# Harrypotterrrr/DVD-GAN

Measured on AMD Instinct MI355X. Metric: clips/sec per G+Ds+Dt step, 48x64x64 UCF-101 synth, higher is better.
Workload: dtype bf16; 1 GPU; UCF-101-shaped 101-class 48x64x64 clips, G+Ds+Dt hinge step, ch=32, k_sample=8, batch 64/GPU (BASELINE configs[1]); global_batch=64, parallelism=dp1

## Files before the change

dvd_gan_amd/csrc/conv_gb.hip:

```cpp
#include "conv_common.h"

namespace {

#ifndef DVD_GB_EPI_DEEP
#define DVD_GB_EPI_DEEP 0
#endif

constexpr unsigned kRowOOB = 0x80000000u, kStepOOB = 0x40000000u, kRangeCap = 0x3fffffffu;

template <int TM, int WN, int WMV, bool UP2> struct HaloGbCfg {
    static constexpr int PITCH = HaloGeo<UP2>::PITCH;
    static constexpr int NWAVE = WMV * WN;
    static constexpr int PH = WMV * TM * 2;
    static constexpr int HG = UP2 ? ((PH / 2 + 3) * PITCH + 15) / 16 : ((PH + 4) * PITCH + 15) / 16;
    static constexpr int HBYTES = HG * 1024;
    static constexpr int EPI = NWAVE * 32 * 64 * 4;
    static constexpr int LDSB = 2 * HBYTES + 1024 > EPI ? 2 * HBYTES + 1024 : EPI;
};

template <int TM, bool RELU, class LdA, class Next>
__device__ __forceinline__ void gb_step(f32x16 (&acc)[TM][2], const bf16x8 (&b)[2][2], LdA ldA, Next next) {
    constexpr int NU = 2 * TM;
#ifndef DVD_GB_ADEPTH
#define DVD_GB_ADEPTH 2
#endif
    constexpr int AD = DVD_GB_ADEPTH;
    bf16x8 a[NU];
#pragma unroll
    for (int u = 0; u < AD && u < NU; ++u) a[u] = ldA(u);
    __builtin_amdgcn_sched_barrier(0);
#pragma unroll
    for (int u = 0; u < NU; ++u) {
        if (u + AD < NU) a[u + AD] = ldA(u + AD);
        const int kk = u / TM, tm = u % TM;
        if constexpr (RELU) a[u] = __builtin_bit_cast(bf16x8, relu16_bf16(__builtin_bit_cast(u32x4, a[u])));
#pragma unroll
        for (int tn = 0; tn < 2; ++tn)
            acc[tm][tn] = __builtin_amdgcn_mfma_f32_32x32x16_bf16(a[u], b[kk][tn], acc[tm][tn], 0, 0, 0);
        __builtin_amdgcn_sched_barrier(0);
        if (u == 0) {
#ifndef DVD_EXP_NODMA
            next();
#endif
            __builtin_amdgcn_sched_barrier(0);
        }
    }
}

template <int TM, int WN, int WMV, bool RELU, bool UP2, int KS>
__device__ __forceinline__ void conv_halo_gb_tile(const ConvK& p, char* const smem, const int mt, const int nt, const int z, const int ltile) {
    using T = bf16_t;
    using G = HaloGeo<UP2>;
    using Cfg = HaloGbCfg<TM, WN, WMV, UP2>;
    constexpr int NWAVE = Cfg::NWAVE;
    constexpr int PITCH = G::PITCH;
    constexpr int BNt = WN * 64;
    constexpr int PH = Cfg::PH, HG = Cfg::HG, HBYTES = Cfg::HBYTES;
    constexpr int NH = (HG + NWAVE - 1) / NWAVE;
    constexpr int ntap2 = KS * KS;
    constexpr int pad = KS >> 1, cpad = (pad + 1) >> 1;
    constexpr int HWa = UP2 ? ((15 + pad) >> 1) + cpad + 1 : 16 + 2 * pad;
    constexpr int HHa = UP2 ? ((PH - 1 + pad) >> 1) + cpad + 1 : PH + 2 * pad;
    char* const hbuf0 = &smem[0];
    char* const dump = &smem[2 * HBYTES];
    const int tid = threadIdx.x, lane = tid & 63, wave = tid >> 6;
    const int wm = wave / WN, wn = wave % WN;
    const int n0 = nt * BNt;
    const int pw = p.W >> 4, ppf = pw * (p.H / PH);
    const int ft = mt / ppf, pidx = mt - ft * ppf;
    const int y0 = (pidx / pw) * PH, x0 = (pidx % pw) * 16;
    const int nouter = p.kchunks * p.kt;
    const int per = (nouter + p.nsplit - 1) / p.nsplit;
    const int oc_begin = z * per, oc_end = min(nouter, oc_begin + per);
    constexpr unsigned esz = 2;
    const int iy_lo = UP2 ? (y0 >> 1) - cpad : y0 - pad, ix_lo = UP2 ? (x0 >> 1) - cpad : x0 - pad;

    const int wu = __builtin_amdgcn_readfirstlane(wave);
    const int lrow = lane >> 2;
    const unsigned ldb = (unsigned)p.ldi * esz;
    const int tt = p.kt > 1 ? ft % p.T : 0;
    const int base_frame = max(0, ft - (p.kt >> 1));
    const size_t fbytes = (size_t)p.Hin * p.Win * ldb;
    const size_t base_b = (size_t)base_frame * fbytes;
    const size_t left_b = p.in_bytes - base_b;
    const __amdgpu_buffer_rsrc_t rin = __builtin_amdgcn_make_buffer_rsrc(
        (void*)(p.in + base_b), 0, left_b > kRangeCap ? kRangeCap : (unsigned)left_b, 0x00020000);
    const int nb32 = p.nb32;
    const __amdgpu_buffer_rsrc_t rwq = __builtin_amdgcn_make_buffer_rsrc(
        (void*)p.wq, 0, (unsigned)((size_t)p.kt * ntap2 * p.kchunks * nb32 * 2048), 0x00020000);
    auto hrow = [&](int i, int& hy, int& hx) __attribute__((always_inline)) {
        const int h = (i * NWAVE + wu) * 16 + lrow;
        hy = h / PITCH; hx = h - hy * PITCH;
    };
    unsigned hoff[NH];
#pragma unroll
    for (int i = 0; i < NH; ++i) {
        const int g = i * NWAVE + wu;
        int hy, hx;
        hrow(i, hy, hx);
        const int yin = iy_lo + hy, xin = ix_lo + hx;
        const int hq = (lane & 3) ^ G::sw(hy, hx);
        const bool ok = g < HG && hy < HHa && hx < HWa && (unsigned)yin < (unsigned)p.Hin && (unsigned)xin < (unsigned)p.Win;
        hoff[i] = ok ? (unsigned)(yin * p.Win + xin) * ldb + hq * 16 : kRowOOB;
    }
    const bool ragged = (p.C & 31) != 0;
    auto dmaH = [&](int hb, int cc_, int it_) __attribute__((always_inline)) {
        const int dt_ = it_ - (p.kt >> 1);
        const bool ok_ = (unsigned)(tt + dt_) < (unsigned)p.T || p.kt == 1;
        const unsigned ud_ = ok_ ? (unsigned)(ft + dt_ - base_frame) * (unsigned)fbytes + cc_ * 64 : kStepOOB;
        const bool part_ = ragged && cc_ == p.kchunks - 1;
#pragma unroll
        for (int i = 0; i < NH; ++i) {
            const int g = i * NWAVE + wu;
            char* dst_ = g < HG ? hbuf0 + hb * HBYTES + g * 1024 : dump;
            unsigned off_ = hoff[i] + ud_;
            if (part_) {
                int hy, hx;
                hrow(i, hy, hx);
                const int hq = (lane & 3) ^ G::sw(hy, hx);
                off_ = cc_ * 32 + hq * 8 < p.C ? off_ : kRowOOB;
            }
            dma16(rin, dst_, off_);
        }
    };
    const unsigned bvoff = (unsigned)(wn * 2 * 2048 + lane * 16);
    const unsigned bnt = (unsigned)(nt * (BNt / 32)) * 2048u;
    const unsigned brec = (unsigned)nb32 * 2048u;
    const unsigned tapstep = (unsigned)p.kchunks * brec;
    auto ldBq = [&](bf16x8 (&b)[2][2], unsigned rec) __attribute__((always_inline)) {
#pragma unroll
        for (int kk = 0; kk < 2; ++kk)
#pragma unroll
            for (int tn = 0; tn < 2; ++tn)
                b[kk][tn] = __builtin_bit_cast(bf16x8, __builtin_amdgcn_raw_buffer_load_b128(rwq, bvoff, rec + (unsigned)(tn * 2048 + kk * 1024), 0));
    };
    auto rec0 = [&](int cc_, int it_) __attribute__((always_inline)) -> unsigned {
        return ((unsigned)(it_ * ntap2) * p.kchunks + cc_) * brec + bnt;
    };

    f32x16 acc[TM][2];
    {
        const f32x16 zacc = {0.f, 0.f, 0.f, 0.f, 0.f, 0.f, 0.f, 0.f, 0.f, 0.f, 0.f, 0.f, 0.f, 0.f, 0.f, 0.f};
#pragma unroll
        for (int a = 0; a < TM; ++a)
#pragma unroll
            for (int b = 0; b < 2; ++b) acc[a][b] = zacc;
    }
    const int l31 = lane & 31, kh2 = lane >> 5;
    const int px = l31 & 15, py0 = wm * (TM * 2) + (l31 >> 4);
    constexpr int TMSTRIDE = (UP2 ? 1 : 2) * PITCH * 64;
#ifdef DVD_EXP_NOMAIN
    const int nouter_z = 0;
#else
    const int nouter_z = oc_end - oc_begin;
#endif
    if (nouter_z > 0) {
        int m_cc = oc_begin / p.kt, m_it = oc_begin - m_cc * p.kt;
        int h_cc = m_cc, h_it = m_it;
        bf16x8 bq0[2][2], bq1[2][2];
        unsigned rec = rec0(m_cc, m_it);
        dmaH(0, h_cc, h_it);
        if (++h_it == p.kt) { h_it = 0; ++h_cc; }
        ldBq(bq0, rec);
        __builtin_amdgcn_s_waitcnt(0x0070 | (0xf << 8));
        __builtin_amdgcn_s_barrier();
        int hb = 0, iy = 0, left = nouter_z;
        auto row = [&](bf16x8 (&b0)[2][2], bf16x8 (&b1)[2][2]) __attribute__((always_inline)) {
            const bool first = iy == 0, last = iy == KS - 1, more = left > 1;
            const int hy = UP2 ? ((py0 + iy - pad) >> 1) + cpad : py0 + iy;
            const char* const Arow = hbuf0 + hb * HBYTES + hy * (PITCH * 64);
#pragma unroll
            for (int ix = 0; ix < KS; ++ix) {
                const int hx = UP2 ? ((px + ix - pad) >> 1) + cpad : px + ix;
                const int swz = G::sw(hy, hx);
                const char* const Ah = Arow + hx * 64;
                auto ldA = [&](int u) __attribute__((always_inline)) -> bf16x8 {
                    const int kk = u / TM, tm = u % TM, slot = kk * 2 + kh2;
                    const int sl = (UP2 && (tm & 1)) ? (slot ^ 2) : slot;
                    return *reinterpret_cast<const bf16x8*>(Ah + tm * TMSTRIDE + ((sl ^ swz) << 4));
                };
                unsigned nrec = rec + tapstep;
                if (ix == KS - 1 && last) {
                    int n_cc = m_cc, n_it = m_it + 1;
                    if (n_it == p.kt) { n_it = 0; ++n_cc; }
                    nrec = more ? rec0(n_cc, n_it) : rec;
                    m_cc = n_cc; m_it = n_it;
                }
                auto next = [&]() __attribute__((always_inline)) {
                    ldBq((ix & 1) ? b0 : b1, nrec);
                    if (ix == 0 && first && more) { dmaH(hb ^ 1, h_cc, h_it); if (++h_it == p.kt) { h_it = 0; ++h_cc; } }
                };
                gb_step<TM, RELU>(acc, (ix & 1) ? b1 : b0, ldA, next);
                rec = nrec;
            }
            ++iy;
            if (last) {
                iy = 0; hb ^= 1; --left;
                if (more) {
#ifndef DVD_EXP_NOWAIT
                    __builtin_amdgcn_s_waitcnt(0xc07f);
#endif
#ifndef DVD_EXP_NOBAR
                    __builtin_amdgcn_s_barrier();
#endif
                }
            }
        };
        const int nrows = nouter_z * KS;
        int r = 0;
#pragma unroll 1
        for (; r + 1 < nrows; r += 2) { row(bq0, bq1); row(bq1, bq0); }
        if (r < nrows) row(bq0, bq1);
    }
    __syncthreads();

    float* ep = reinterpret_cast<float*>(&smem[0]) + wave * (32 * 64);
    const int ecol = (lane & 7) * 8, erow = lane >> 3;
    const long long frame_row0 = (long long)ft * (p.H * p.W);
    conv_epilogue<T, TM, DVD_GB_EPI_DEEP>(p, acc, ep, lane, n0 + wn * 64 + ecol, z, ltile, frame_row0, [&](int tm, int j) __attribute__((always_inline)) {
        const int pi = wm * (TM * 32) + tm * 32 + j * 8 + erow;
        return (y0 + (pi >> 4)) * p.W + x0 + (pi & 15);
    });
}

__device__ __forceinline__ int xcd_order(int bid, int nwg) {
    const int xcd = bid & 7, qd = nwg >> 3, rr = nwg & 7;
    return (xcd < rr ? xcd * (qd + 1) : rr * (qd + 1) + (xcd - rr) * qd) + (bid >> 3);
}
struct TileMN { int mt, nt; };
__device__ __forceinline__ TileMN tile_of(int nmajor, int tilesN, int t, int ntiles) {
    const int d = nmajor ? ntiles / tilesN : tilesN;
    const int q = t / d, r = t - q * d;
    TileMN o;
    o.mt = nmajor ? r : q; o.nt = nmajor ? q : r;
    return o;
}

template <int TM, int WN, int WMV, bool RELU, bool UP2, int KS>
__global__ __launch_bounds__(256, 2) void conv_halo_gb_kernel(ConvK p) {
    __shared__ __attribute__((aligned(16))) char smem[HaloGbCfg<TM, WN, WMV, UP2>::LDSB];
    const int bid = xcd_order(blockIdx.x, gridDim.x);
    const TileMN t = tile_of(p.nmajor, p.tilesN, bid, gridDim.x);
    conv_halo_gb_tile<TM, WN, WMV, RELU, UP2, KS>(p, smem, t.mt, t.nt, blockIdx.z, (int)blockIdx.x);
}

template <int TM, int S> struct HaloGbsCfg {
    static constexpr int PITCH = S + 4, FR = PITCH * PITCH;
    static constexpr int G = TM * 64 / (S * S);
    static constexpr int HG = (G * FR + 15) / 16;
    static constexpr int HBYTES = HG * 1024;
    static constexpr int EPI = 4 * 32 * 64 * 4;
    static constexpr int LDSB = 2 * HBYTES + 1024 > EPI ? 2 * HBYTES + 1024 : EPI;
};

template <int TM, int S, bool RELU, int KS>
__device__ __forceinline__ void conv_halo_gbs_tile(const ConvK& p, char* const smem, const int mt, const int nt, const int z, const int ltile) {
    using T = bf16_t;
    using Cfg = HaloGbsCfg<TM, S>;
    constexpr int WN = 2, NWAVE = 4, BNt = 128;
    constexpr int PITCH = Cfg::PITCH, FR = Cfg::FR, G = Cfg::G, HG = Cfg::HG, HBYTES = Cfg::HBYTES;
    constexpr int NH = (HG + NWAVE - 1) / NWAVE;
    constexpr int SS = S * S;
    constexpr int ntap2 = KS * KS, pad = KS >> 1, ext = S + 2 * pad;
    char* const hbuf0 = &smem[0];
    char* const dump = &smem[2 * HBYTES];
    const int tid = threadIdx.x, lane = tid & 63, wave = tid >> 6;
    const int wm = wave / WN, wn = wave % WN;
    const int n0 = nt * BNt;
    const int ft0 = mt * G, nframes = p.M / SS;
    const int per = (p.kchunks + p.nsplit - 1) / p.nsplit;
    const int cc_begin = z * per, cc_end = min(p.kchunks, cc_begin + per);
    constexpr unsigned esz = 2;

    const int wu = __builtin_amdgcn_readfirstlane(wave);
    const int lrow = lane >> 2;
    const unsigned ldb = (unsigned)p.ldi * esz;
    const size_t base_b = (size_t)ft0 * SS * ldb;
    const size_t left_b = p.in_bytes - base_b;
    const __amdgpu_buffer_rsrc_t rin = __builtin_amdgcn_make_buffer_rsrc(
        (void*)(p.in + base_b), 0, left_b > kRangeCap ? kRangeCap : (unsigned)left_b, 0x00020000);
    const int nb32 = p.nb32;
    const __amdgpu_buffer_rsrc_t rwq = __builtin_amdgcn_make_buffer_rsrc(
        (void*)p.wq, 0, (unsigned)((size_t)ntap2 * p.kchunks * nb32 * 2048), 0x00020000);
    auto hrow = [&](int i, int& fl, int& hy, int& hx) __attribute__((always_inline)) {
        const int h = (i * NWAVE + wu) * 16 + lrow;
        fl = h / FR;
        const int r = h - fl * FR;
        hy = r / PITCH; hx = r - hy * PITCH;
    };
    unsigned hoff[NH];
#pragma unroll
    for (int i = 0; i < NH; ++i) {
        const int g = i * NWAVE + wu;
        int fl, hy, hx;
        hrow(i, fl, hy, hx);
        const int yin = hy - pad, xin = hx - pad;
        const int hq = (lane & 3) ^ (hy & 3);
        const bool ok = g < HG && fl < G && ft0 + fl < nframes && hy < ext && hx < ext && (unsigned)yin < (unsigned)S && (unsigned)xin < (unsigned)S;
        hoff[i] = ok ? (unsigned)((fl * S + yin) * S + xin) * ldb + hq * 16 : kRowOOB;
    }
    const bool ragged = (p.C & 31) != 0;
    auto dmaH = [&](int hb, int cc_) __attribute__((always_inline)) {
        const bool part_ = ragged && cc_ == p.kchunks - 1;
#pragma unroll
        for (int i = 0; i < NH; ++i) {
            const int g = i * NWAVE + wu;
            char* dst_ = g < HG ? hbuf0 + hb * HBYTES + g * 1024 : dump;
            unsigned off_ = hoff[i] + cc_ * 64;
            if (part_) {
                int fl, hy, hx;
                hrow(i, fl, hy, hx);
                const int hq = (lane & 3) ^ (hy & 3);
                off_ = cc_ * 32 + hq * 8 < p.C ? off_ : kRowOOB;
            }
            dma16(rin, dst_, off_);
        }
    };
    const unsigned bvoff = (unsigned)(wn * 2 * 2048 + lane * 16);
    const unsigned bnt = (unsigned)(nt * (BNt / 32)) * 2048u;
    const unsigned brec = (unsigned)nb32 * 2048u;
    const unsigned tapstep = (unsigned)p.kchunks * brec;
    auto ldBq = [&](bf16x8 (&b)[2][2], unsigned rec) __attribute__((always_inline)) {
#pragma unroll
        for (int kk = 0; kk < 2; ++kk)
#pragma unroll
            for (int tn = 0; tn < 2; ++tn)
                b[kk][tn] = __builtin_bit_cast(bf16x8, __builtin_amdgcn_raw_buffer_load_b128(rwq, bvoff, rec + (unsigned)(tn * 2048 + kk * 1024), 0));
    };

    f32x16 acc[TM][2];
    {
        const f32x16 zacc = {0.f, 0.f, 0.f, 0.f, 0.f, 0.f, 0.f, 0.f, 0.f, 0.f, 0.f, 0.f, 0.f, 0.f, 0.f, 0.f};
#pragma unroll
        for (int a = 0; a < TM; ++a)
#pragma unroll
            for (int b = 0; b < 2; ++b) acc[a][b] = zacc;
    }
    const int l31 = lane & 31, kh2 = lane >> 5;
    const int pi0 = wm * (TM * 32) + l31;
    const int f0 = pi0 / SS, y0 = (pi0 % SS) / S, x0 = pi0 % S;
    const int arow0 = f0 * FR + y0 * PITCH + x0;
    auto tmoff = [](int tm) constexpr -> int { return S == 8 ? ((tm >> 1) * FR + (tm & 1) * 4 * PITCH) * 64 : tm * 2 * FR * 64; };
#ifdef DVD_EXP_NOMAIN
    const int nch = 0;
#else
    const int nch = cc_end - cc_begin;
#endif
    if (nch > 0) {
        unsigned rec = (unsigned)cc_begin * brec + bnt;
        bf16x8 bq0[2][2], bq1[2][2];
        dmaH(0, cc_begin);
        ldBq(bq0, rec);
        __builtin_amdgcn_s_waitcnt(0x0070 | (0xf << 8));
        __builtin_amdgcn_s_barrier();
        int hb = 0, iy = 0, cc = cc_begin;
        auto row = [&](bf16x8 (&b0)[2][2], bf16x8 (&b1)[2][2]) __attribute__((always_inline)) {
            const bool first = iy == 0, last = iy == KS - 1, more = cc + 1 < cc_end;
            const int swz = (y0 + iy) & 3;
            const char* const Arow = hbuf0 + hb * HBYTES + (arow0 + iy * PITCH) * 64;
#pragma unroll
            for (int ix = 0; ix < KS; ++ix) {
                const char* const Ah = Arow + ix * 64;
                auto ldA = [&](int u) __attribute__((always_inline)) -> bf16x8 {
                    const int kk = u / TM, tm = u % TM, slot = kk * 2 + kh2;
                    return *reinterpret_cast<const bf16x8*>(Ah + tmoff(tm) + ((slot ^ swz) << 4));
                };
                unsigned nrec = rec + tapstep;
                if (ix == KS - 1 && last) nrec = more ? (unsigned)(cc + 1) * brec + bnt : rec;
                auto next = [&]() __attribute__((always_inline)) {
                    ldBq((ix & 1) ? b0 : b1, nrec);
                    if (ix == 0 && first && more) dmaH(hb ^ 1, cc + 1);
                };
                gb_step<TM, RELU>(acc, (ix & 1) ? b1 : b0, ldA, next);
                rec = nrec;
            }
            ++iy;
            if (last) {
                iy = 0; hb ^= 1; ++cc;
                if (more) {
                    __builtin_amdgcn_s_waitcnt(0xc07f);
                    __builtin_amdgcn_s_barrier();
                }
            }
        };
        const int nrows = nch * KS;
        int r = 0;
#pragma unroll 1
        for (; r + 1 < nrows; r += 2) { row(bq0, bq1); row(bq1, bq0); }
        if (r < nrows) row(bq0, bq1);
    }
    __syncthreads();

    float* ep = reinterpret_cast<float*>(&smem[0]) + wave * (32 * 64);
    const int ecol = (lane & 7) * 8, erow = lane >> 3;
    const long long row0 = (long long)ft0 * SS;
    conv_epilogue<T, TM, DVD_GB_EPI_DEEP>(p, acc, ep, lane, n0 + wn * 64 + ecol, z, ltile, row0, [&](int tm, int j) __attribute__((always_inline)) {
        const int pi = wm * (TM * 32) + tm * 32 + j * 8 + erow;
        return row0 + pi < p.M ? pi : -1;
    });
}

template <int TM, int S, bool RELU, int KS>
__global__ __launch_bounds__(256, 2) void conv_halo_gbs_kernel(ConvK p) {
    __shared__ __attribute__((aligned(16))) char smem[HaloGbsCfg<TM, S>::LDSB];
    const int bid = xcd_order(blockIdx.x, gridDim.x);
    const TileMN t = tile_of(p.nmajor, p.tilesN, bid, gridDim.x);
    conv_halo_gbs_tile<TM, S, RELU, KS>(p, smem, t.mt, t.nt, blockIdx.z, (int)blockIdx.x);
}

template <class TileFn>
__device__ __forceinline__ void group_dispatch(const ConvGroup& grp, TileFn fn) {
    const int x = blockIdx.x & 7;
    int rem = blockIdx.x >> 3;
    auto share = [&](int m) __attribute__((always_inline)) -> int { const int w = grp.wgs[m]; return (w >> 3) + (x < (w & 7) ? 1 : 0); };
    const int m0 = grp.order[0], m1 = grp.n > 1 ? grp.order[1] : m0;
    const int s0 = share(m0), s1 = grp.n > 1 ? share(m1) : 0;
    const int h0 = min(grp.head, s0), h1 = min(grp.head, s1);
    int g = -1, off = 0;
    if (rem < h0) { g = m0; off = rem; }
    else if ((rem -= h0) < h1) { g = m1; off = rem; }
    else if ((rem -= h1) < s0 - h0) { g = m0; off = h0 + rem; }
    else if ((rem -= s0 - h0) < s1 - h1) { g = m1; off = h1 + rem; }
    else {
        rem -= s1 - h1;
        for (int k = 2; k < grp.n; ++k) {
            const int m = grp.order[k], s = share(m);
            if (rem < s) { g = m; off = rem; break; }
            rem -= s;
        }
    }
    if (g < 0) return;
    const int w = grp.wgs[g];
    const int local = x * (w >> 3) + min(x, w & 7) + off;
    const ConvK& p = grp.c[g];
    const int t = local / p.nsplit, z = local - t * p.nsplit;
    const TileMN mn = tile_of(p.nmajor, p.tilesN, t, w / p.nsplit);
    fn(p, mn.mt, mn.nt, z, t);
}

template <int TM, int WN, int WMV>
__global__ __launch_bounds__(256, 2) void conv_group_gb_kernel(ConvGroup grp) {
    __shared__ __attribute__((aligned(16))) char smem[HaloGbCfg<TM, WN, WMV, false>::LDSB];
    group_dispatch(grp, [&](const ConvK& p, int mt, int nt, int z, int t) __attribute__((always_inline)) {
        if (p.kh == 5) conv_halo_gb_tile<TM, WN, WMV, false, false, 5>(p, smem, mt, nt, z, t);
        else conv_halo_gb_tile<TM, WN, WMV, false, false, 3>(p, smem, mt, nt, z, t);
    });
}

template <int TM, int S>
__global__ __launch_bounds__(256, 2) void conv_group_gbs_kernel(ConvGroup grp) {
    __shared__ __attribute__((aligned(16))) char smem[HaloGbsCfg<TM, S>::LDSB];
    group_dispatch(grp, [&](const ConvK& p, int mt, int nt, int z, int t) __attribute__((always_inline)) {
        if (p.kh == 5) conv_halo_gbs_tile<TM, S, false, 5>(p, smem, mt, nt, z, t);
        else conv_halo_gbs_tile<TM, S, false, 3>(p, smem, mt, nt, z, t);
    });
}

}

namespace dvdk {
#define GB(R, C, KS, RL, UP) cv_key(CV_HALO_L2, 0, R, C, KS, RL, UP)
#define GBS(F, R, KS, RL) cv_key(F, 0, R, 128, KS, RL, 0)
static const ConvRow kGbRows[] = {
#ifdef DVD_GB_PROBE
    {GB(256, 128, 5, 0, 0), conv_halo_gb_kernel<4, 2, 2, false, false, 5>}, {GBS(CV_FRAME8, 128, 3, 0), conv_halo_gbs_kernel<2, 8, false, 3>},
#else
    {GB(256, 128, 3, 0, 0), conv_halo_gb_kernel<4, 2, 2, false, false, 3>}, {GB(256, 128, 3, 1, 0), conv_halo_gb_kernel<4, 2, 2, true, false, 3>},
    {GB(256, 128, 3, 0, 1), conv_halo_gb_kernel<4, 2, 2, false, true, 3>},  {GB(256, 128, 3, 1, 1), conv_halo_gb_kernel<4, 2, 2, true, true, 3>},
    {GB(256, 128, 5, 0, 0), conv_halo_gb_kernel<4, 2, 2, false, false, 5>}, {GB(256, 128, 5, 1, 0), conv_halo_gb_kernel<4, 2, 2, true, false, 5>},
    {GB(256, 128, 5, 0, 1), conv_halo_gb_kernel<4, 2, 2, false, true, 5>},  {GB(256, 128, 5, 1, 1), conv_halo_gb_kernel<4, 2, 2, true, true, 5>},
    {GB(128, 128, 3, 0, 0), conv_halo_gb_kernel<2, 2, 2, false, false, 3>}, {GB(128, 128, 3, 1, 0), conv_halo_gb_kernel<2, 2, 2, true, false, 3>},
    {GB(128, 128, 3, 0, 1), conv_halo_gb_kernel<2, 2, 2, false, true, 3>},  {GB(128, 128, 3, 1, 1), conv_halo_gb_kernel<2, 2, 2, true, true, 3>},
    {GB(128, 128, 5, 0, 0), conv_halo_gb_kernel<2, 2, 2, false, false, 5>}, {GB(128, 128, 5, 1, 0), conv_halo_gb_kernel<2, 2, 2, true, false, 5>},
    {GB(128, 128, 5, 0, 1), conv_halo_gb_kernel<2, 2, 2, false, true, 5>},  {GB(128, 128, 5, 1, 1), conv_halo_gb_kernel<2, 2, 2, true, true, 5>},
    {GB(256, 64, 3, 0, 0), conv_halo_gb_kernel<2, 1, 4, false, false, 3>},  {GB(256, 64, 3, 1, 0), conv_halo_gb_kernel<2, 1, 4, true, false, 3>},
    {GB(256, 64, 3, 0, 1), conv_halo_gb_kernel<2, 1, 4, false, true, 3>},   {GB(256, 64, 3, 1, 1), conv_halo_gb_kernel<2, 1, 4, true, true, 3>},
    {GB(256, 64, 5, 0, 0), conv_halo_gb_kernel<2, 1, 4, false, false, 5>},  {GB(256, 64, 5, 1, 0), conv_halo_gb_kernel<2, 1, 4, true, false, 5>},
    {GB(256, 64, 5, 0, 1), conv_halo_gb_kernel<2, 1, 4, false, true, 5>},   {GB(256, 64, 5, 1, 1), conv_halo_gb_kernel<2, 1, 4, true, true, 5>},
    {GBS(CV_FRAME8, 256, 3, 0), conv_halo_gbs_kernel<4, 8, false, 3>},      {GBS(CV_FRAME8, 256, 3, 1), conv_halo_gbs_kernel<4, 8, true, 3>},
    {GBS(CV_FRAME8, 256, 5, 0), conv_halo_gbs_kernel<4, 8, false, 5>},      {GBS(CV_FRAME8, 256, 5, 1), conv_halo_gbs_kernel<4, 8, true, 5>},
    {GBS(CV_FRAME8, 128, 3, 0), conv_halo_gbs_kernel<2, 8, false, 3>},      {GBS(CV_FRAME8, 128, 3, 1), conv_halo_gbs_kernel<2, 8, true, 3>},
    {GBS(CV_FRAME8, 128, 5, 0), conv_halo_gbs_kernel<2, 8, false, 5>},      {GBS(CV_FRAME8, 128, 5, 1), conv_halo_gbs_kernel<2, 8, true, 5>},
    {GBS(CV_FRAME4, 128, 3, 0), conv_halo_gbs_kernel<2, 4, false, 3>},      {GBS(CV_FRAME4, 128, 3, 1), conv_halo_gbs_kernel<2, 4, true, 3>},
    {GBS(CV_FRAME4, 128, 5, 0), conv_halo_gbs_kernel<2, 4, false, 5>},      {GBS(CV_FRAME4, 128, 5, 1), conv_halo_gbs_kernel<2, 4, true, 5>},
#endif
};
#undef GB
#undef GBS
bool launch_gb(unsigned key, const ConvK& p, dim3 grid, hipStream_t st) { return cv_launch_row(kGbRows, (int)(sizeof kGbRows / sizeof kGbRows[0]), key, p, grid, 256, st); }
static void (*const kGroupKernel[])(ConvGroup) = {
#ifdef DVD_GB_PROBE
    conv_group_gb_kernel<4, 2, 2>, conv_group_gb_kernel<4, 2, 2>, conv_group_gb_kernel<4, 2, 2>, conv_group_gb_kernel<4, 2, 2>, conv_group_gb_kernel<4, 2, 2>,
#else
    conv_group_gb_kernel<4, 2, 2>, conv_group_gb_kernel<2, 2, 2>, conv_group_gbs_kernel<4, 8>, conv_group_gbs_kernel<2, 8>, conv_group_gbs_kernel<2, 4>,
#endif
};
static_assert(sizeof kGroupKernel / sizeof kGroupKernel[0] == kGroupKinds, "one kernel per row of kGroupKind");
void launch_group(const ConvGroup& grp, int kind, hipStream_t st) { kGroupKernel[kind]<<<dim3(grp.nslots), 256, 0, st>>>(grp); }
}
```

Measured before the change: 145.1 clips/s.

## Remap small-frame conv tiles to whole image lines and skip all-padding tap rows

Reorganizes the small-frame (S=4/8) halo conv kernel so each 32-row MFMA sub-tile covers whole image lines across frames, using a new compile-time row map. With that layout, per-wave kernel-row ranges and per-row sub-tile masks are computed at compile time, so MFMAs and B loads for taps that only read zero padding are skipped. The chunk loop is fully unrolled per wave-row with a triple-buffered B register set and wave-specific specializations. The changes are meant to remove wasted MFMA work on padding at small spatial sizes, at the cost of more code size, register pressure and a changed LDS swizzle and epilogue mapping.

```diff
diff --git a/dvd_gan_amd/csrc/conv_gb.hip b/dvd_gan_amd/csrc/conv_gb.hip
--- a/dvd_gan_amd/csrc/conv_gb.hip
+++ b/dvd_gan_amd/csrc/conv_gb.hip
@@ -1,10 +1,18 @@
+#include <type_traits>
+#include <utility>
+
 #include "conv_common.h"
+#include "gbs_rowmap.h"
 
 namespace {
 
 #ifndef DVD_GB_EPI_DEEP
 #define DVD_GB_EPI_DEEP 0
 #endif
+
+template <class F, int... I>
+__device__ __forceinline__ void static_for_seq(F&& f, std::integer_sequence<int, I...>) { (f(std::integral_constant<int, I>{}), ...); }
+template <int N, class F> __device__ __forceinline__ void static_for(F&& f) { static_for_seq(f, std::make_integer_sequence<int, N>{}); }
 
 constexpr unsigned kRowOOB = 0x80000000u, kStepOOB = 0x40000000u, kRangeCap = 0x3fffffffu;
 
@@ -18,21 +26,22 @@
     static constexpr int LDSB = 2 * HBYTES + 1024 > EPI ? 2 * HBYTES + 1024 : EPI;
 };
 
-template <int TM, bool RELU, class LdA, class Next>
+template <int TM, int T0, int NT, bool RELU, class LdA, class Next>
 __device__ __forceinline__ void gb_step(f32x16 (&acc)[TM][2], const bf16x8 (&b)[2][2], LdA ldA, Next next) {
-    constexpr int NU = 2 * TM;
+    static_assert(T0 >= 0 && NT >= 1 && T0 + NT <= TM, "sub-tile range");
+    constexpr int NU = 2 * NT;
 #ifndef DVD_GB_ADEPTH
 #define DVD_GB_ADEPTH 2
 #endif
     constexpr int AD = DVD_GB_ADEPTH;
     bf16x8 a[NU];
 #pragma unroll
-    for (int u = 0; u < AD && u < NU; ++u) a[u] = ldA(u);
+    for (int u = 0; u < AD && u < NU; ++u) a[u] = ldA(u / NT, T0 + u % NT);
     __builtin_amdgcn_sched_barrier(0);
 #pragma unroll
     for (int u = 0; u < NU; ++u) {
-        if (u + AD < NU) a[u + AD] = ldA(u + AD);
-        const int kk = u / TM, tm = u % TM;
+        if (u + AD < NU) a[u + AD] = ldA((u + AD) / NT, T0 + (u + AD) % NT);
+        const int kk = u / NT, tm = T0 + u % NT;
         if constexpr (RELU) a[u] = __builtin_bit_cast(bf16x8, relu16_bf16(__builtin_bit_cast(u32x4, a[u])));
 #pragma unroll
         for (int tn = 0; tn < 2; ++tn)
@@ -174,8 +183,8 @@
                 const int hx = UP2 ? ((px + ix - pad) >> 1) + cpad : px + ix;
                 const int swz = G::sw(hy, hx);
                 const char* const Ah = Arow + hx * 64;
-                auto ldA = [&](int u) __attribute__((always_inline)) -> bf16x8 {
-                    const int kk = u / TM, tm = u % TM, slot = kk * 2 + kh2;
+                auto ldA = [&](int kk, int tm) __attribute__((always_inline)) -> bf16x8 {
+                    const int slot = kk * 2 + kh2;
                     const int sl = (UP2 && (tm & 1)) ? (slot ^ 2) : slot;
                     return *reinterpret_cast<const bf16x8*>(Ah + tm * TMSTRIDE + ((sl ^ swz) << 4));
                 };
@@ -190,7 +199,7 @@
                     ldBq((ix & 1) ? b0 : b1, nrec);
                     if (ix == 0 && first && more) { dmaH(hb ^ 1, h_cc, h_it); if (++h_it == p.kt) { h_it = 0; ++h_cc; } }
                 };
-                gb_step<TM, RELU>(acc, (ix & 1) ? b1 : b0, ldA, next);
+                gb_step<TM, 0, TM, RELU>(acc, (ix & 1) ? b1 : b0, ldA, next);
                 rec = nrec;
             }
             ++iy;
@@ -257,6 +266,8 @@
 __device__ __forceinline__ void conv_halo_gbs_tile(const ConvK& p, char* const smem, const int mt, const int nt, const int z, const int ltile) {
     using T = bf16_t;
     using Cfg = HaloGbsCfg<TM, S>;
+    using Map = GbsMap<TM, S>;
+    static_assert(Map::PITCH == Cfg::PITCH && Map::FR == Cfg::FR && Map::G == Cfg::G, "one geometry");
     constexpr int WN = 2, NWAVE = 4, BNt = 128;
     constexpr int PITCH = Cfg::PITCH, FR = Cfg::FR, G = Cfg::G, HG = Cfg::HG, HBYTES = Cfg::HBYTES;
     constexpr int NH = (HG + NWAVE - 1) / NWAVE;
@@ -295,7 +306,7 @@
         int fl, hy, hx;
         hrow(i, fl, hy, hx);
         const int yin = hy - pad, xin = hx - pad;
-        const int hq = (lane & 3) ^ (hy & 3);
+        const int hq = (lane & 3) ^ Map::swz(fl, hy);
         const bool ok = g < HG && fl < G && ft0 + fl < nframes && hy < ext && hx < ext && (unsigned)yin < (unsigned)S && (unsigned)xin < (unsigned)S;
         hoff[i] = ok ? (unsigned)((fl * S + yin) * S + xin) * ldb + hq * 16 : kRowOOB;
     }
@@ -310,7 +321,7 @@
             if (part_) {
                 int fl, hy, hx;
                 hrow(i, fl, hy, hx);
-                const int hq = (lane & 3) ^ (hy & 3);
+                const int hq = (lane & 3) ^ Map::swz(fl, hy);
                 off_ = cc_ * 32 + hq * 8 < p.C ? off_ : kRowOOB;
             }
             dma16(rin, dst_, off_);
@@ -337,57 +348,67 @@
             for (int b = 0; b < 2; ++b) acc[a][b] = zacc;
     }
     const int l31 = lane & 31, kh2 = lane >> 5;
-    const int pi0 = wm * (TM * 32) + l31;
-    const int f0 = pi0 / SS, y0 = (pi0 % SS) / S, x0 = pi0 % S;
-    const int arow0 = f0 * FR + y0 * PITCH + x0;
-    auto tmoff = [](int tm) constexpr -> int { return S == 8 ? ((tm >> 1) * FR + (tm & 1) * 4 * PITCH) * 64 : tm * 2 * FR * 64; };
+    const int f0 = Map::frame(l31), y0 = Map::line(wm * TM, l31);
+    const int arow0 = Map::arow(wm * TM, l31);
+    auto tmoff = [](int tm) constexpr -> int { return tm * Map::LPS * PITCH * 64; };
 #ifdef DVD_EXP_NOMAIN
     const int nch = 0;
 #else
     const int nch = cc_end - cc_begin;
 #endif
     if (nch > 0) {
-        unsigned rec = (unsigned)cc_begin * brec + bnt;
-        bf16x8 bq0[2][2], bq1[2][2];
+        const int wmu = wu / WN;
+        const int iy_lo = wmu ? Map::row_lo(1, KS) : Map::row_lo(0, KS);
+        const unsigned rbase = bnt + (unsigned)(iy_lo * KS) * tapstep;
+        unsigned rec = (unsigned)cc_begin * brec + rbase;
+        bf16x8 bq[3][2][2];
         dmaH(0, cc_begin);
-        ldBq(bq0, rec);
+        ldBq(bq[0], rec);
         __builtin_amdgcn_s_waitcnt(0x0070 | (0xf << 8));
         __builtin_amdgcn_s_barrier();
-        int hb = 0, iy = 0, cc = cc_begin;
-        auto row = [&](bf16x8 (&b0)[2][2], bf16x8 (&b1)[2][2]) __attribute__((always_inline)) {
-            const bool first = iy == 0, last = iy == KS - 1, more = cc + 1 < cc_end;
-            const int swz = (y0 + iy) & 3;
-            const char* const Arow = hbuf0 + hb * HBYTES + (arow0 + iy * PITCH) * 64;
-#pragma unroll
-            for (int ix = 0; ix < KS; ++ix) {
-                const char* const Ah = Arow + ix * 64;
-                auto ldA = [&](int u) __attribute__((always_inline)) -> bf16x8 {
-                    const int kk = u / TM, tm = u % TM, slot = kk * 2 + kh2;
-                    return *reinterpret_cast<const bf16x8*>(Ah + tmoff(tm) + ((slot ^ swz) << 4));
-                };
-                unsigned nrec = rec + tapstep;
-                if (ix == KS - 1 && last) nrec = more ? (unsigned)(cc + 1) * brec + bnt : rec;
-                auto next = [&]() __attribute__((always_inline)) {
-                    ldBq((ix & 1) ? b0 : b1, nrec);
-                    if (ix == 0 && first && more) dmaH(hb ^ 1, cc + 1);
-                };
-                gb_step<TM, RELU>(acc, (ix & 1) ? b1 : b0, ldA, next);
-                rec = nrec;
-            }
-            ++iy;
-            if (last) {
-                iy = 0; hb ^= 1; ++cc;
-                if (more) {
-                    __builtin_amdgcn_s_waitcnt(0xc07f);
-                    __builtin_amdgcn_s_barrier();
-                }
+        int hb = 0, cc = cc_begin;
+        auto chunk = [&](auto wmc) __attribute__((always_inline)) {
+            constexpr int WM = decltype(wmc)::value;
+            constexpr int ILO = Map::row_lo(WM, KS), NV = Map::row_hi(WM, KS) - ILO + 1, NS = NV * KS;
+            const bool more = cc + 1 < cc_end;
+            const char* const Abuf = hbuf0 + hb * HBYTES + arow0 * 64;
+            static_for<NV>([&](auto rc) __attribute__((always_inline)) {
+                constexpr int iy = ILO + decltype(rc)::value;
+                constexpr unsigned m = Map::row_mask(WM, iy, KS);
+                constexpr int T0 = Map::mask_t0(m), NT = Map::mask_nt(m);
+                static_assert(NT >= 1 && m == ((1u << NT) - 1) << T0, "a row's sub-tiles are a contiguous run");
+                const int swz = Map::swz(f0, y0 + iy);
+                static_for<KS>([&](auto xc) __attribute__((always_inline)) {
+                    constexpr int ix = decltype(xc)::value, s = decltype(rc)::value * KS + ix;
+                    constexpr int cur = gbs_bset(s, NS), nxt = gbs_bset((s + 1) % NS, NS);
+                    const char* const Ah = Abuf + (iy * PITCH + ix) * 64;
+                    auto ldA = [&](int kk, int tm) __attribute__((always_inline)) -> bf16x8 {
+                        const int slot = kk * 2 + kh2;
+                        return *reinterpret_cast<const bf16x8*>(Ah + tmoff(tm) + ((slot ^ swz) << 4));
+                    };
+                    unsigned nrec = rec + tapstep;
+                    if (s == NS - 1) nrec = more ? (unsigned)(cc + 1) * brec + rbase : rec;
+                    auto next = [&]() __attribute__((always_inline)) {
+                        ldBq(bq[nxt], nrec);
+                        if (s == 0 && more) dmaH(hb ^ 1, cc + 1);
+                    };
+                    gb_step<TM, T0, NT, RELU>(acc, bq[cur], ldA, next);
+                    rec = nrec;
+                });
+            });
+            hb ^= 1; ++cc;
+            if (more) {
+                __builtin_amdgcn_s_waitcnt(0xc07f);
+                __builtin_amdgcn_s_barrier();
             }
         };
-        const int nrows = nch * KS;
-        int r = 0;
+        if (wmu == 0) {
 #pragma unroll 1
-        for (; r + 1 < nrows; r += 2) { row(bq0, bq1); row(bq1, bq0); }
-        if (r < nrows) row(bq0, bq1);
+            for (int c = 0; c < nch; ++c) chunk(std::integral_constant<int, 0>{});
+        } else {
+#pragma unroll 1
+            for (int c = 0; c < nch; ++c) chunk(std::integral_constant<int, 1>{});
+        }
     }
     __syncthreads();
 
@@ -395,7 +416,7 @@
     const int ecol = (lane & 7) * 8, erow = lane >> 3;
     const long long row0 = (long long)ft0 * SS;
     conv_epilogue<T, TM, DVD_GB_EPI_DEEP>(p, acc, ep, lane, n0 + wn * 64 + ecol, z, ltile, row0, [&](int tm, int j) __attribute__((always_inline)) {
-        const int pi = wm * (TM * 32) + tm * 32 + j * 8 + erow;
+        const int pi = Map::rel(wm * TM + tm, j * 8 + erow);
         return row0 + pi < p.M ? pi : -1;
     });
 }
@@ -464,6 +485,7 @@
 static const ConvRow kGbRows[] = {
 #ifdef DVD_GB_PROBE
     {GB(256, 128, 5, 0, 0), conv_halo_gb_kernel<4, 2, 2, false, false, 5>}, {GBS(CV_FRAME8, 128, 3, 0), conv_halo_gbs_kernel<2, 8, false, 3>},
+    {GBS(CV_FRAME8, 256, 5, 0), conv_halo_gbs_kernel<4, 8, false, 5>},      {GBS(CV_FRAME4, 128, 5, 0), conv_halo_gbs_kernel<2, 4, false, 5>},
 #else
     {GB(256, 128, 3, 0, 0), conv_halo_gb_kernel<4, 2, 2, false, false, 3>}, {GB(256, 128, 3, 1, 0), conv_halo_gb_kernel<4, 2, 2, true, false, 3>},
     {GB(256, 128, 3, 0, 1), conv_halo_gb_kernel<4, 2, 2, false, true, 3>},  {GB(256, 128, 3, 1, 1), conv_halo_gb_kernel<4, 2, 2, true, true, 3>},
diff --git a/dvd_gan_amd/csrc/gbs_rowmap.h b/dvd_gan_amd/csrc/gbs_rowmap.h
--- /dev/null
+++ b/dvd_gan_amd/csrc/gbs_rowmap.h
@@ -0,0 +1,52 @@
+#pragma once
+
+#if defined(__HIPCC__)
+#define GBS_HD __host__ __device__
+#else
+#define GBS_HD
+#endif
+
+template <int TM, int S> struct GbsMap {
+    static constexpr int PITCH = S + 4, FR = PITCH * PITCH, SS = S * S;
+    static constexpr int G = TM * 64 / SS;
+    static constexpr int NSUB = 2 * TM;
+    static constexpr int LPS = S / NSUB;
+    static_assert(LPS >= 1 && LPS * NSUB == S && G * S * LPS == 32, "a sub-tile is whole image lines of all frames");
+
+    static GBS_HD constexpr int frame(int l) { return l / (S * LPS); }
+    static GBS_HD constexpr int line(int sub, int l) { return sub * LPS + (l / S) % LPS; }
+    static GBS_HD constexpr int col(int l) { return l % S; }
+    static GBS_HD constexpr int rel(int sub, int l) { return frame(l) * SS + line(sub, l) * S + col(l); }
+    static GBS_HD constexpr int arow(int sub, int l) { return frame(l) * FR + line(sub, l) * PITCH + col(l); }
+    static GBS_HD constexpr int swz(int f, int hy) { return (f * LPS + hy % LPS) & 3; }
+    static GBS_HD constexpr unsigned row_mask(int wm, int iy, int KS) {
+        unsigned m = 0;
+        for (int tm = 0; tm < TM; ++tm) {
+            const int lo = (wm * TM + tm) * LPS + iy - KS / 2;
+            if (lo + LPS - 1 >= 0 && lo < S) m |= 1u << tm;
+        }
+        return m;
+    }
+    static GBS_HD constexpr int row_lo(int wm, int KS) {
+        int i = 0;
+        while (i < KS && !row_mask(wm, i, KS)) ++i;
+        return i;
+    }
+    static GBS_HD constexpr int row_hi(int wm, int KS) {
+        int i = KS - 1;
+        while (i >= 0 && !row_mask(wm, i, KS)) --i;
+        return i;
+    }
+    static GBS_HD constexpr int mask_t0(unsigned m) {
+        int t = 0;
+        while (t < TM && !(m >> t & 1u)) ++t;
+        return t;
+    }
+    static GBS_HD constexpr int mask_nt(unsigned m) {
+        int n = 0;
+        for (int t = 0; t < TM; ++t) n += (int)(m >> t & 1u);
+        return n;
+    }
+};
+
+GBS_HD constexpr int gbs_bset(int s, int n) { return (n & 1) && s == n - 1 ? 2 : s & 1; }
```

Measured after the change: 145.9 clips/s, median of 6. No clear change (+0.6%).
